# HueCodes/sudoku-vision

Hardware: AMD Instinct MI355X
Metric: end-to-end frames/sec (1080p->81 digits) (higher is better)
Workload: dtype f32

## Files before the change

sudoku-vision_amd/csrc/k2_cells_body.h:

```cpp
#pragma once
#include "sv_device.h"

namespace sv_k2 {

constexpr int OUT = 450, CELL = 50, MARGIN = 5, CROP = 40, CS = 28;

struct CellsLds {
    u8 crop[CROP * CROP];
    int tab[CS][3];
    double M[9];
    double org[CROP][2][3];
};

__device__ __forceinline__ int resize_px(const u8 *crop, int cw, int sh, int sw, int xo, int xa0, int xa1, int yo, int b0, int b1)
{
    int sx = xo, a0 = xa0, a1 = xa1;
    if (sx < 0) { sx = 0; a0 = 2048; a1 = 0; }
    if (sx >= sw - 1) { sx = sw - 1; a0 = 2048; a1 = 0; }
    const int sx1 = sx + 1 < sw ? sx + 1 : sx;
    const int sy0 = sv_clamp(yo, 0, sh - 1), sy1 = sv_clamp(yo + 1, 0, sh - 1);
    const int t0 = crop[sy0 * cw + sx] * a0 + crop[sy0 * cw + sx1] * a1;
    const int t1 = crop[sy1 * cw + sx] * a0 + crop[sy1 * cw + sx1] * a1;
    return (((b0 * (t0 >> 4)) >> 16) + ((b1 * (t1 >> 4)) >> 16) + 2) >> 2;
}

__device__ __forceinline__ void warp_cells_item(const u8 *__restrict__ frames, int H, int W, ptrdiff_t pitch, ptrdiff_t frame_stride,
                                                const double *__restrict__ minv, u8 *__restrict__ cells, int frame, int cell, CellsLds &L)
{
    const int tid = threadIdx.x;
    const int r = cell / 9, c = cell - r * 9;
    const u8 *img = frames + (ptrdiff_t)frame * frame_stride;
    if (tid < 9) L.M[tid] = minv[(ptrdiff_t)frame * 9 + tid];
    if (tid >= 64 && tid < 64 + CS) {
        int o, w0, w1;
        sv_resize_axis(CROP, CS, tid - 64, o, w0, w1);
        L.tab[tid - 64][0] = o;
        L.tab[tid - 64][1] = w0;
        L.tab[tid - 64][2] = w1;
    }
    __syncthreads();

    const int bw = sv_warp_block_w(OUT, OUT);
    const int xlo = c * CELL + MARGIN, ylo = r * CELL + MARGIN, blk0 = xlo / bw;
    if (tid < 2 * CROP) {
        const int y = tid >> 1, k = tid & 1;
        sv_warp_block_origin(L.M, (blk0 + k) * bw, ylo + y, L.org[y][k][0], L.org[y][k][1], L.org[y][k][2]);
    }
    __syncthreads();
    for (int i = tid; i < CROP * CROP; i += 256) {
        const int y = i / CROP, x = i - y * CROP;
        const int dx = xlo + x, k = dx / bw - blk0;
        int sx, sy, a, b, px[3];
        sv_warp_coord_from(L.M, L.org[y][k][0], L.org[y][k][1], L.org[y][k][2], dx - (blk0 + k) * bw, sx, sy, a, b);
        sv_warp_sample<3>(img, H, W, pitch, sx, sy, a, b, px);
        L.crop[i] = (u8)sv_gray_px(px[0], px[1], px[2]);
    }
    __syncthreads();

    u8 *dst = cells + ((ptrdiff_t)frame * 81 + cell) * (CS * CS);
    for (int i = tid; i < CS * CS; i += 256) {
        const int y = i / CS, x = i - y * CS;
        dst[i] = (u8)resize_px(L.crop, CROP, CROP, CROP, L.tab[x][0], L.tab[x][1], L.tab[x][2], L.tab[y][0], L.tab[y][1], L.tab[y][2]);
    }
}

}
```

sudoku-vision_amd/csrc/sv_device.h:

```cpp
#pragma once
#include <hip/hip_runtime.h>
#include <cstdint>

typedef uint8_t u8;

__device__ __forceinline__ int sv_gray_px(int b, int g, int r)
{
    return (b * 3735 + g * 19235 + r * 9798 + 16384) >> 15;
}

__device__ __forceinline__ int sv_clamp(int v, int lo, int hi) { return v < lo ? lo : (v > hi ? hi : v); }

__device__ __forceinline__ float sv_glue_norm(u8 c)
{
    const float t = __fdiv_rn((float)(255 - (int)c), 255.0f);
    return __fdiv_rn(__fsub_rn(t, 0.5f), 0.5f);
}

__device__ __forceinline__ int sv_reflect101(int p, int len)
{
    if (len == 1) return 0;
    while (p < 0 || p >= len) p = p < 0 ? -p : 2 * len - 2 - p;
    return p;
}

__host__ __device__ __forceinline__ int sv_warp_block_w(int dw, int dh)
{
    int bh0 = 16 < dh ? 16 : dh;
    int bw0 = 1024 / bh0 < dw ? 1024 / bh0 : dw;
    return bw0;
}

__device__ __forceinline__ void sv_warp_block_origin(const double *M, int x0, int dy, double &X0, double &Y0, double &W0)
{
    const double fx0 = (double)x0, fy = (double)dy;
    X0 = __dadd_rn(__dadd_rn(__dmul_rn(M[0], fx0), __dmul_rn(M[1], fy)), M[2]);
    Y0 = __dadd_rn(__dadd_rn(__dmul_rn(M[3], fx0), __dmul_rn(M[4], fy)), M[5]);
    W0 = __dadd_rn(__dadd_rn(__dmul_rn(M[6], fx0), __dmul_rn(M[7], fy)), M[8]);
}

__device__ __forceinline__ void sv_warp_coord_from(const double *M, double X0, double Y0, double W0, int x1, int &sx, int &sy, int &a, int &b)
{
    const double fx1 = (double)x1;
    double Wv = __dadd_rn(W0, __dmul_rn(M[6], fx1));
    Wv = Wv != 0.0 ? __ddiv_rn(32.0, Wv) : 0.0;
    double fX = __dmul_rn(__dadd_rn(X0, __dmul_rn(M[0], fx1)), Wv);
    double fY = __dmul_rn(__dadd_rn(Y0, __dmul_rn(M[3], fx1)), Wv);
    fX = fmax(-2147483648.0, fmin(2147483647.0, fX));
    fY = fmax(-2147483648.0, fmin(2147483647.0, fY));
    const int X = __double2int_rn(fX), Y = __double2int_rn(fY);
    sx = sv_clamp(X >> 5, -32768, 32767);
    sy = sv_clamp(Y >> 5, -32768, 32767);
    a = X & 31;
    b = Y & 31;
}

__device__ __forceinline__ void sv_warp_coord(const double *M, int dx, int dy, int bw, int &sx, int &sy, int &a, int &b)
{
    const int x0 = (dx / bw) * bw;
    double X0, Y0, W0;
    sv_warp_block_origin(M, x0, dy, X0, Y0, W0);
    sv_warp_coord_from(M, X0, Y0, W0, dx - x0, sx, sy, a, b);
}

__device__ __forceinline__ int sv_tap(const u8 *img, int H, int W, ptrdiff_t pitch, int C, int x, int y, int c)
{
    if ((unsigned)x >= (unsigned)W || (unsigned)y >= (unsigned)H) return 0;
    return img[(ptrdiff_t)y * pitch + (ptrdiff_t)x * C + c];
}

template <int C>
__device__ __forceinline__ void sv_warp_sample(const u8 *img, int H, int W, ptrdiff_t pitch, int sx, int sy, int a, int b, int (&out)[C]);

template <int C>
__device__ __forceinline__ void sv_warp_px(const u8 *img, int H, int W, ptrdiff_t pitch, const double *M, int dx, int dy,
                                           int bw, int (&out)[C])
{
    int sx, sy, a, b;
    sv_warp_coord(M, dx, dy, bw, sx, sy, a, b);
    sv_warp_sample<C>(img, H, W, pitch, sx, sy, a, b, out);
}

template <int C>
__device__ __forceinline__ void sv_warp_sample(const u8 *img, int H, int W, ptrdiff_t pitch, int sx, int sy, int a, int b, int (&out)[C])
{
    const int w00 = (32 - a) * (32 - b) * 32, w01 = a * (32 - b) * 32, w10 = (32 - a) * b * 32, w11 = a * b * 32;
    const bool inside = (unsigned)sx < (unsigned)(W - 1) && (unsigned)sy < (unsigned)(H - 1);
    if (inside) {
        const u8 *p0 = img + (ptrdiff_t)sy * pitch + (ptrdiff_t)sx * C;
        const u8 *p1 = p0 + pitch;
#pragma unroll
        for (int c = 0; c < C; c++)
            out[c] = (p0[c] * w00 + p0[C + c] * w01 + p1[c] * w10 + p1[C + c] * w11 + 16384) >> 15;
    } else {
#pragma unroll
        for (int c = 0; c < C; c++)
            out[c] = (sv_tap(img, H, W, pitch, C, sx, sy, c) * w00 + sv_tap(img, H, W, pitch, C, sx + 1, sy, c) * w01 +
                      sv_tap(img, H, W, pitch, C, sx, sy + 1, c) * w10 + sv_tap(img, H, W, pitch, C, sx + 1, sy + 1, c) * w11 +
                      16384) >> 15;
    }
}

__device__ __forceinline__ void sv_resize_axis_scaled(double scale, int d, int &ofs, int &w0, int &w1)
{
    float f = (float)__dadd_rn(__dmul_rn(__dadd_rn((double)d, 0.5), scale), -0.5);
    const int s = (int)floorf(f);
    f = __fsub_rn(f, (float)s);
    ofs = s;
    w0 = __float2int_rn(__fmul_rn(__fsub_rn(1.f, f), 2048.f));
    w1 = __float2int_rn(__fmul_rn(f, 2048.f));
}

__device__ __forceinline__ void sv_resize_axis(int s_len, int d_len, int d, int &ofs, int &w0, int &w1)
{
    sv_resize_axis_scaled(__ddiv_rn(1.0, __ddiv_rn((double)d_len, (double)s_len)), d, ofs, w0, w1);
}

template <int NTHREADS>
__device__ __forceinline__ void sv_fc2_stage(float (*w2s)[128], const float *w2, int tid)
{
    for (int i = tid; i < 1280; i += NTHREADS) w2s[i >> 7][i & 127] = w2[i];
}

__device__ __forceinline__ float sv_fc2_logit(const float *h, const float (*w2s)[128], const float *b2, int j)
{
    float s = b2[j];
    for (int n = 0; n < 128; n++) s = __builtin_fmaf(h[n], w2s[j][n], s);
    return s;
}

__device__ __forceinline__ int sv_argmax10(const float *lg, float &best)
{
    best = lg[0];
    int arg = 0;
    for (int j = 1; j < 10; j++)
        if (lg[j] > best) { best = lg[j]; arg = j; }
    return arg;
}

__device__ __forceinline__ void sv_digit_conf(const float *lg, long cell, u8 *digits, float *conf)
{
    if (!digits && !conf) return;
    float best;
    const int arg = sv_argmax10(lg, best);
    if (digits) digits[cell] = (u8)arg;
    if (conf) {
        float den = 0.f;
        for (int j = 0; j < 10; j++) den += expf(lg[j] - best);
        conf[cell] = 1.0f / den;
    }
}

__device__ __forceinline__ void sv_digit_conf_t(const float *lg, float temperature, long cell, u8 *digits, float *conf)
{
    if (!digits && !conf) return;
    float best;
    const int arg = sv_argmax10(lg, best);
    if (digits) digits[cell] = (u8)arg;
    if (conf) {
        best = best / temperature;
        float den = 0.f;
        for (int j = 0; j < 10; j++) den += expf(lg[j] / temperature - best);
        conf[cell] = 1.0f / den;
    }
}
```

Baseline: 196,900.

## Speed up cell-crop warp sampling with fast reciprocal, packed loads and dot4

Rewrites the crop-fill loop of the cells kernel. The exact double division in the perspective warp is replaced by a hardware reciprocal with one Newton step, and a proof check falls back to the exact path wave-wide whenever rounding could be ambiguous. Each pixel loads two unaligned 64-bit rows and computes the horizontal bilinear blend with udot4 byte dot products. The loop is software-pipelined so the next pixel's address and loads are issued before the current one is blended. This adds code complexity and relies on unaligned 8-byte loads staying inside the frame buffer, guarded by a width check.

```diff
diff --git a/sudoku-vision_amd/csrc/k2_cells_body.h b/sudoku-vision_amd/csrc/k2_cells_body.h
--- a/sudoku-vision_amd/csrc/k2_cells_body.h
+++ b/sudoku-vision_amd/csrc/k2_cells_body.h
@@ -24,6 +24,102 @@
     return (((b0 * (t0 >> 4)) >> 16) + ((b1 * (t1 >> 4)) >> 16) + 2) >> 2;
 }
 
+typedef unsigned long long __attribute__((aligned(1))) u64_any;
+
+struct CropPx {
+    int sx, sy, a, b;
+    bool wide;
+    unsigned long long r0, r1;
+
+    __device__ __forceinline__ void locate(const CellsLds &L, const u8 *img, int H, int W, unsigned pitch32, double M0, double M3, double M6,
+                                           int x, int y, int xsplit, int bw)
+    {
+        const int k = x >= xsplit;
+        const double *o = L.org[y][k];
+        const double fx1 = (double)(x - xsplit + (k ? 0 : bw));
+        const double Xn = __dadd_rn(o[0], __dmul_rn(M0, fx1)), Yn = __dadd_rn(o[1], __dmul_rn(M3, fx1)), Wd = __dadd_rn(o[2], __dmul_rn(M6, fx1));
+        int X, Y;
+        const bool proven = sv_warp_xy_fast(Xn, Yn, Wd, X, Y);
+        if (__any(!proven)) sv_warp_xy_exact(Xn, Yn, Wd, X, Y);
+        sv_warp_cell_frac(X, Y, sx, sy, a, b);
+        wide = (unsigned)sx < (unsigned)(W - 2) && (unsigned)sy < (unsigned)(H - 1);
+        const u8 *p = img + ((unsigned long long)(wide ? (unsigned)sy : 0u) * pitch32 + (wide ? (unsigned)(sx * 3) : 0u));
+        r0 = *(const u64_any *)p;
+        r1 = *(const u64_any *)(p + pitch32);
+    }
+
+    static __device__ __forceinline__ void row_h(unsigned long long r, unsigned wa, int (&h)[3])
+    {
+        const unsigned lo = (unsigned)r, hi = (unsigned)(r >> 32);
+        h[0] = (int)__builtin_amdgcn_udot4(lo, wa, 0u, false);
+        h[1] = (int)__builtin_amdgcn_udot4(__builtin_amdgcn_alignbyte(hi, lo, 1), wa, 0u, false);
+        h[2] = (int)__builtin_amdgcn_udot4(__builtin_amdgcn_alignbyte(hi, lo, 2), wa, 0u, false);
+    }
+
+    __device__ __forceinline__ int gray(const u8 *img, int H, int W, ptrdiff_t pitch) const
+    {
+        int px[3];
+        if (wide) {
+            const unsigned wa = (unsigned)(32 - a) | ((unsigned)a << 24);
+            int h0[3], h1[3];
+            row_h(r0, wa, h0);
+            row_h(r1, wa, h1);
+#pragma unroll
+            for (int c = 0; c < 3; c++) px[c] = (int)((__umul24(32 - b, h0[c]) + __umul24(b, h1[c]) + 512u) >> 10);
+            return (int)((__umul24(px[0], 3735) + __umul24(px[1], 19235) + __umul24(px[2], 9798) + 16384u) >> 15);
+        }
+        sv_warp_sample<3>(img, H, W, pitch, sx, sy, a, b, px);
+        return sv_gray_px(px[0], px[1], px[2]);
+    }
+};
+
+__device__ __forceinline__ void crop_step(int &x, int &y)
+{
+    y += 256 / CROP;
+    x += 256 % CROP;
+    if (x >= CROP) { x -= CROP; y++; }
+}
+
+__device__ __forceinline__ void crop_fill(CellsLds &L, const u8 *img, int H, int W, ptrdiff_t pitch, int xlo, int blk0, int bw)
+{
+    const int tid = threadIdx.x;
+    if (W < 3 || H < 2 || pitch <= 0 || pitch > 0x7fffffff) {
+        for (int i = tid; i < CROP * CROP; i += 256) {
+            const int y = i / CROP, x = i - y * CROP;
+            const int dx = xlo + x, k = dx / bw - blk0;
+            int sx, sy, a, b, px[3];
+            sv_warp_coord_from(L.M, L.org[y][k][0], L.org[y][k][1], L.org[y][k][2], dx - (blk0 + k) * bw, sx, sy, a, b);
+            sv_warp_sample<3>(img, H, W, pitch, sx, sy, a, b, px);
+            L.crop[i] = (u8)sv_gray_px(px[0], px[1], px[2]);
+        }
+        return;
+    }
+    const double M0 = L.M[0], M3 = L.M[3], M6 = L.M[6];
+    const int xsplit = (blk0 + 1) * bw - xlo;
+    const unsigned pitch32 = (unsigned)pitch;
+    const int rounds = (CROP * CROP - __builtin_amdgcn_readfirstlane(tid) + 255) / 256;
+    int y = tid / CROP, x = tid - y * CROP;
+    CropPx p, q;
+    int i = tid, j = 1;
+    p.locate(L, img, H, W, pitch32, M0, M3, M6, x, y, xsplit, bw);
+    for (; j + 1 < rounds; j += 2, i += 512) {
+        crop_step(x, y);
+        q.locate(L, img, H, W, pitch32, M0, M3, M6, x, y, xsplit, bw);
+        L.crop[i] = (u8)p.gray(img, H, W, pitch);
+        crop_step(x, y);
+        p.locate(L, img, H, W, pitch32, M0, M3, M6, x, y, xsplit, bw);
+        L.crop[i + 256] = (u8)q.gray(img, H, W, pitch);
+    }
+    if (j < rounds) {
+        crop_step(x, y);
+        q.locate(L, img, H, W, pitch32, M0, M3, M6, x, y, xsplit, bw);
+        L.crop[i] = (u8)p.gray(img, H, W, pitch);
+        L.crop[i + 256] = (u8)q.gray(img, H, W, pitch);
+    } else {
+        L.crop[i] = (u8)p.gray(img, H, W, pitch);
+    }
+}
+
 __device__ __forceinline__ void warp_cells_item(const u8 *__restrict__ frames, int H, int W, ptrdiff_t pitch, ptrdiff_t frame_stride,
                                                 const double *__restrict__ minv, u8 *__restrict__ cells, int frame, int cell, CellsLds &L)
 {
@@ -47,14 +143,7 @@
         sv_warp_block_origin(L.M, (blk0 + k) * bw, ylo + y, L.org[y][k][0], L.org[y][k][1], L.org[y][k][2]);
     }
     __syncthreads();
-    for (int i = tid; i < CROP * CROP; i += 256) {
-        const int y = i / CROP, x = i - y * CROP;
-        const int dx = xlo + x, k = dx / bw - blk0;
-        int sx, sy, a, b, px[3];
-        sv_warp_coord_from(L.M, L.org[y][k][0], L.org[y][k][1], L.org[y][k][2], dx - (blk0 + k) * bw, sx, sy, a, b);
-        sv_warp_sample<3>(img, H, W, pitch, sx, sy, a, b, px);
-        L.crop[i] = (u8)sv_gray_px(px[0], px[1], px[2]);
-    }
+    crop_fill(L, img, H, W, pitch, xlo, blk0, bw);
     __syncthreads();
 
     u8 *dst = cells + ((ptrdiff_t)frame * 81 + cell) * (CS * CS);
diff --git a/sudoku-vision_amd/csrc/sv_device.h b/sudoku-vision_amd/csrc/sv_device.h
--- a/sudoku-vision_amd/csrc/sv_device.h
+++ b/sudoku-vision_amd/csrc/sv_device.h
@@ -39,20 +39,45 @@
     W0 = __dadd_rn(__dadd_rn(__dmul_rn(M[6], fx0), __dmul_rn(M[7], fy)), M[8]);
 }
 
-__device__ __forceinline__ void sv_warp_coord_from(const double *M, double X0, double Y0, double W0, int x1, int &sx, int &sy, int &a, int &b)
+__device__ __forceinline__ void sv_warp_xy_exact(double Xn, double Yn, double Wd, int &X, int &Y)
 {
-    const double fx1 = (double)x1;
-    double Wv = __dadd_rn(W0, __dmul_rn(M[6], fx1));
-    Wv = Wv != 0.0 ? __ddiv_rn(32.0, Wv) : 0.0;
-    double fX = __dmul_rn(__dadd_rn(X0, __dmul_rn(M[0], fx1)), Wv);
-    double fY = __dmul_rn(__dadd_rn(Y0, __dmul_rn(M[3], fx1)), Wv);
+    const double Wv = Wd != 0.0 ? __ddiv_rn(32.0, Wd) : 0.0;
+    double fX = __dmul_rn(Xn, Wv);
+    double fY = __dmul_rn(Yn, Wv);
     fX = fmax(-2147483648.0, fmin(2147483647.0, fX));
     fY = fmax(-2147483648.0, fmin(2147483647.0, fY));
-    const int X = __double2int_rn(fX), Y = __double2int_rn(fY);
+    X = __double2int_rn(fX);
+    Y = __double2int_rn(fY);
+}
+
+#define SV_WARP_TIE 0x1p-18
+__device__ __forceinline__ bool sv_warp_xy_fast(double Xn, double Yn, double Wd, int &X, int &Y)
+{
+    const double r0 = __builtin_amdgcn_rcp(Wd);
+    const double e = __builtin_fma(-Wd, r0, 1.0);
+    const double q = __dmul_rn(__builtin_fma(r0, e, r0), 32.0);
+    const double tX = __dmul_rn(Xn, q), tY = __dmul_rn(Yn, q);
+    const double rX = rint(tX), rY = rint(tY);
+    X = (int)rX;
+    Y = (int)rY;
+    const double dX = fabs(__dsub_rn(tX, rX)), dY = fabs(__dsub_rn(tY, rY));
+    return (int)(fabs(Wd) < 0x1p1000) & (int)(fabs(tX) < 0x1p22) & (int)(fabs(tY) < 0x1p22) & (int)(dX < 0.5 - SV_WARP_TIE) & (int)(dY < 0.5 - SV_WARP_TIE);
+}
+
+__device__ __forceinline__ void sv_warp_cell_frac(int X, int Y, int &sx, int &sy, int &a, int &b)
+{
     sx = sv_clamp(X >> 5, -32768, 32767);
     sy = sv_clamp(Y >> 5, -32768, 32767);
     a = X & 31;
     b = Y & 31;
+}
+
+__device__ __forceinline__ void sv_warp_coord_from(const double *M, double X0, double Y0, double W0, int x1, int &sx, int &sy, int &a, int &b)
+{
+    const double fx1 = (double)x1;
+    int X, Y;
+    sv_warp_xy_exact(__dadd_rn(X0, __dmul_rn(M[0], fx1)), __dadd_rn(Y0, __dmul_rn(M[3], fx1)), __dadd_rn(W0, __dmul_rn(M[6], fx1)), X, Y);
+    sv_warp_cell_frac(X, Y, sx, sy, a, b);
 }
 
 __device__ __forceinline__ void sv_warp_coord(const double *M, int dx, int dy, int bw, int &sx, int &sy, int &a, int &b)
```

New measurement: 195,800, median of 3. No clear change (-0.6%).
